# rcelha/rio-rs

Measured on NVIDIA H100. Metric: placements/sec, higher is better.
Workload: dtype u32

## Files before the change

rio_rs_b200/csrc/engine.cu:

```cuda
#include "../../include/rio_cuda.h"
#include "../../include/rio_cuda_dev.h"
#include "kernels.cuh"
#include "k_ranked.cuh"
#include "k_affinity_ranked.cuh"
#include "k_changes.cuh"
#include "k_ranked_changes.cuh"
#include "spec.cuh"
#include "trie_table.hpp"

#include <dlfcn.h>

#include <algorithm>
#include <atomic>
#include <chrono>
#include <cstdio>
#include <cstring>
#include <mutex>
#include <string>
#include <unordered_map>
#include <vector>

using namespace rio;

namespace {
// ... 190 lines not shown
    return h->h_scalars[which];
}
void check_device_error(rio_placement *h) {
    uint32_t e = 0;
    CUDA_TRY(cudaMemcpyAsync(&e, h->d_error(), 4, cudaMemcpyDeviceToHost, h->stream));
    CUDA_TRY(cudaStreamSynchronize(h->stream));
    if (e) { CUDA_TRY(cudaMemsetAsync(h->d_error(), 0, 4, h->stream)); throw RioError{RIO_ERR_UNKNOWN, "directory table overflow (internal sizing error)"}; }
}

bool address_malformed(const std::string &a) {
    size_t c = a.find(':');
    return c == std::string::npos || c == 0 || c + 1 >= a.size();
}

uint32_t intern_node(rio_placement *h, const std::string &addr) {
    auto it = h->node_index.find(addr);
    if (it != h->node_index.end()) return it->second;
    REQUIRE(h->nodes.size() < 0xFFFFFFF0u, "too many nodes");
    NodeInfo ni;
    ni.addr = addr;
    ni.seed = mix64(fnv1a64(addr.data(), addr.size()));
    ni.seed2 = mix64(ni.seed ^ kSaltNode2);
    ni.malformed = address_malformed(addr);
    uint32_t idx = (uint32_t)h->nodes.size();
    h->nodes.push_back(std::move(ni));
    h->node_index.emplace(addr, idx);
    h->tab_dirty = true;
    return idx;
}

void build_tab(rio_placement *h, TabBufs &tb, const std::vector<uint8_t> *closed) {
    const uint32_t n_total = (uint32_t)h->nodes.size();
    struct Ent { uint32_t invw, idx; };
    std::vector<Ent> live;
    auto is_closed = [&](uint32_t j) { return closed && j < closed->size() && (*closed)[j]; };
    for (uint32_t j = 0; j < n_total; j++) {
        const NodeInfo &ni = h->nodes[j];
        if (!ni.live()) continue;
        if (is_closed(j)) continue;
        live.push_back(Ent{inv_weight(ni.weight), j});
    }
    {
        std::vector<uint32_t> classes_seen;
        bool few = true;
        for (const Ent &e : live) {
            if (std::find(classes_seen.begin(), classes_seen.end(), e.invw) != classes_seen.end()) continue;
            if (classes_seen.size() == 64) { few = false; break; }
            classes_seen.push_back(e.invw);
        }
        if (few) {
            std::sort(classes_seen.begin(), classes_seen.end());
            std::vector<uint32_t> start(classes_seen.size() + 1, 0);
            auto cls = [&](uint32_t invw) { return (size_t)(std::lower_bound(classes_seen.begin(), classes_seen.end(), invw) - classes_seen.begin()); };
            for (const Ent &e : live) start[cls(e.invw) + 1]++;
            for (size_t c = 0; c < classes_seen.size(); c++) start[c + 1] += start[c];
            std::vector<Ent> grouped(live.size());
            for (const Ent &e : live) grouped[start[cls(e.invw)]++] = e;
            live.swap(grouped);
        } else {
            std::sort(live.begin(), live.end(), [](const Ent &a, const Ent &b) { return a.invw != b.invw ? a.invw < b.invw : a.idx < b.idx; });
        }
    }
    std::vector<NodeRec> recs(live.size() ? live.size() : 1);
    std::vector<ClassRec> classes;
    for (size_t q = 0; q < live.size(); q++) {
        const NodeInfo &ni = h->nodes[live[q].idx];
        recs[q] = NodeRec{(uint32_t)ni.seed, live[q].idx, (uint32_t)(ni.seed >> 32) | 1u, (uint32_t)ni.seed2};
        if (q == 0 || live[q].invw != live[q - 1].invw || (h->dev_table_flags & RIO_DEV_SPLIT_CLASSES)) classes.push_back(ClassRec{(uint32_t)q, live[q].invw});
    }
    const uint32_t n_classes = (uint32_t)classes.size();
    classes.push_back(ClassRec{(uint32_t)live.size(), 0});
    classes.push_back(ClassRec{(uint32_t)live.size(), 0});
    std::vector<uint4> by_idx(n_total ? n_total : 1);
    for (uint32_t j = 0; j < n_total; j++) {
        const NodeInfo &ni = h->nodes[j];
        const bool lv = ni.live() && !is_closed(j);
        by_idx[j] = make_uint4((uint32_t)ni.seed, lv ? inv_weight(ni.weight) : 0u, (uint32_t)(ni.seed >> 32) | 1u, (uint32_t)ni.seed2);
    }
    std::vector<TrieMember> members;
    members.reserve(live.size());
    for (const Ent &e : live) members.push_back(TrieMember{h->nodes[e.idx].seed, e.idx, h->nodes[e.idx].weight});
    const TrieBlob blob = build_trie_blob(members, h->trie_bits);
    const uint32_t bits = blob.bits, nb = 1u << bits, blob_bytes = blob.blob_bytes;
    std::vector<uint8_t> state(n_total ? n_total : 1, 0);
    std::vector<uint32_t> livef(n_total ? n_total : 1, 0);
    for (uint32_t j = 0; j < n_total; j++) {
        const NodeInfo &ni = h->nodes[j];
        state[j] = ((ni.active && !ni.malformed) ? kNodeLive : 0) | (ni.malformed ? kNodeMalformed : 0);
        livef[j] = ni.live() ? 1u : 0u;
    }

    auto al = [](size_t v) { return (v + 255) & ~(size_t)255; };
    const size_t o_recs = 0, o_classes = al(o_recs + recs.size() * sizeof(NodeRec)), o_byidx = al(o_classes + classes.size() * sizeof(ClassRec)),
                 o_trie = al(o_byidx + by_idx.size() * sizeof(uint4)), o_state = al(o_trie + blob_bytes), o_live = al(o_state + state.size()),
                 total = al(o_live + livef.size() * 4);
    cudaStream_t st = h->stream;
    if (tb.upload_pending) { CUDA_TRY(cudaStreamSynchronize(st)); tb.upload_pending = false; }
    if (h->aux_stream) CUDA_TRY(cudaStreamSynchronize(h->aux_stream));
    if (total > tb.stage_cap) {
        if (tb.stage) CUDA_TRY(cudaFreeHost(tb.stage));
        tb.stage = nullptr; tb.stage_cap = 0;
        CUDA_TRY(cudaMallocHost(reinterpret_cast<void **>(&tb.stage), total * 2));
        tb.stage_cap = total * 2;
    }
    memcpy(tb.stage + o_recs, recs.data(), recs.size() * sizeof(NodeRec));
    memcpy(tb.stage + o_classes, classes.data(), classes.size() * sizeof(ClassRec));
    memcpy(tb.stage + o_byidx, by_idx.data(), by_idx.size() * sizeof(uint4));
    memcpy(tb.stage + o_trie, blob.words.data(), blob_bytes);
    memcpy(tb.stage + o_state, state.data(), state.size());
    memcpy(tb.stage + o_live, livef.data(), livef.size() * 4);
    tb.dev.ensure(total, st);
    CUDA_TRY(cudaMemcpyAsync(tb.dev.p, tb.stage, total, cudaMemcpyHostToDevice, st));
    tb.upload_pending = true;
    unsigned char *d = tb.dev.as<unsigned char>();
    tb.trie = TrieDev{d + o_trie, blob_bytes, blob.off_crec, bits, blob.n_chain, {}};
    for (uint32_t i = 1; i < 8 && i < nb; i++) tb.trie.top[i] = blob.words[i];
    tb.tab.recs = reinterpret_cast<const NodeRec *>(d + o_recs);
    tb.tab.classes = reinterpret_cast<const ClassRec *>(d + o_classes);
    tb.tab.by_idx = reinterpret_cast<const uint4 *>(d + o_byidx);
    tb.tab.n_live = (uint32_t)live.size();
    tb.tab.n_classes = n_classes;
    tb.tab.n_total = n_total;
    tb.state = d + o_state;
    tb.live = reinterpret_cast<const uint32_t *>(d + o_live);
}

uint64_t live_signature(const rio_placement *h) {
    uint64_t sig = kFnvBasis;
    for (uint32_t j = 0; j < (uint32_t)h->nodes.size(); j++)
        if (h->nodes[j].live()) sig = mix64(sig ^ (((uint64_t)j << 32) | h->nodes[j].weight));
    return sig;
}

void ensure_tab(rio_placement *h) {
    if (!h->tab_dirty) return;
    build_tab(h, h->tabs, nullptr);
    const uint32_t n_total = (uint32_t)h->nodes.size();
    cudaStream_t st = h->stream;
    h->tab_dirty = false;
    h->tab_version++;
    h->live_sig = live_signature(h);
    if (!h->K) return;
    std::vector<float> fnode((size_t)(n_total ? n_total : 1) * h->K, 0.f);
    for (uint32_t j = 0; j < n_total; j++) {
        const NodeInfo &ni = h->nodes[j];
        if (ni.feat.size() == h->K) std::copy(ni.feat.begin(), ni.feat.end(), fnode.begin() + (size_t)j * h->K);
    }
    h->d_fnode.ensure(fnode.size() * 4, st);
    CUDA_TRY(cudaMemcpyAsync(h->d_fnode.p, fnode.data(), fnode.size() * 4, cudaMemcpyHostToDevice, st));
    h->aff_live = h->aff_pad = 0;
    if (h->K == 16) {
        std::vector<uint32_t> map;
        for (uint32_t j = 0; j < n_total; j++) if (h->nodes[j].live()) map.push_back(j);
        const uint32_t nl = (uint32_t)map.size();
        const uint32_t pad = nl <= 64 ? 64 : (nl + 255) / 256 * 256;
        std::vector<float> fc((size_t)pad * 16, 0.f);
        for (uint32_t q = 0; q < nl; q++) if (h->nodes[map[q]].feat.size() == 16) std::copy(h->nodes[map[q]].feat.begin(), h->nodes[map[q]].feat.end(), fc.begin() + (size_t)q * 16);
        map.resize(pad, kNone);
        std::vector<float> fg(fc.size());
        for (uint32_t g8 = 0; g8 < pad / 8; g8++)
            for (uint32_t k4 = 0; k4 < 4; k4++)
                for (uint32_t r8 = 0; r8 < 8; r8++)
                    std::copy_n(fc.begin() + ((size_t)g8 * 8 + r8) * 16 + k4 * 4, 4, fg.begin() + (((size_t)g8 * 4 + k4) * 8 + r8) * 4);
        h->d_fnode_c.ensure(fc.size() * 4, st);
        h->d_fnode_g.ensure(fg.size() * 4, st);
        CUDA_TRY(cudaMemcpyAsync(h->d_fnode_g.p, fg.data(), fg.size() * 4, cudaMemcpyHostToDevice, st));
        h->d_nidx_map.ensure(map.size() * 4, st);
        CUDA_TRY(cudaMemcpyAsync(h->d_fnode_c.p, fc.data(), fc.size() * 4, cudaMemcpyHostToDevice, st));
        CUDA_TRY(cudaMemcpyAsync(h->d_nidx_map.p, map.data(), map.size() * 4, cudaMemcpyHostToDevice, st));
        CUDA_TRY(cudaStreamSynchronize(st));
        h->aff_live = nl; h->aff_pad = pad;
    }
    CUDA_TRY(cudaStreamSynchronize(st));
}

uint64_t pow2_at_least(uint64_t v) { uint64_t p = 1; while (p < v) p <<= 1; return p; }

void dir_alloc(rio_placement *h, uint64_t cap, DirDev &out) {
    void *p = nullptr;
    CUDA_TRY(cudaMallocAsync(&p, cap * sizeof(DirSlot), h->stream));
    out.slots = reinterpret_cast<DirSlot *>(p);
    out.mask = cap - 1;
    uint32_t lg = 0; while ((1ull << lg) < cap) lg++;
    out.shift = 64 - lg;
    launch_dir_init(h->L(), out.slots, cap);
}

void reconcile_dir_keys(rio_placement *h) {
    h->dir_keys = read_scalar(h, S_NEWKEYS);
    h->dir_keys_pending = 0;
}

void dir_reserve(rio_placement *h, uint64_t n_more) {
    const uint64_t need = h->dir_keys + h->dir_keys_pending + n_more;
    if (need * 10 <= h->dir_cap * 7) return;
    if (h->dir_keys_pending) { reconcile_dir_keys(h); if ((h->dir_keys + n_more) * 10 <= h->dir_cap * 7) return; }
    zero_scalar(h, S_PLACED);
    launch_dir_count(h->L(), h->dir, h->d_scalars + S_PLACED, nullptr, 0);
// ... 1556 lines not shown
```

rio_rs_b200/csrc/k_trie.cu:

```cuda
#include "kernels.cuh"
#include "spec.cuh"
#include "bounded_tail.cuh"

#include <cstdlib>

namespace rio {

namespace {

#define RIO_COUNT_LAUNCH(L) do { if ((L).launch_counter) ++*(L).launch_counter; } while (0)

constexpr int kTrieThreads = 256;
constexpr uint32_t kMaxLevels = 16;

__constant__ uint32_t c_lvl_s0[kMaxLevels];
__constant__ uint32_t c_lvl_m2[kMaxLevels];
__constant__ uint32_t c_lvl_h2[kMaxLevels];

__device__ __forceinline__ uint32_t smem_u32(const void *p) { return (uint32_t)__cvta_generic_to_shared(p); }

__device__ __forceinline__ void stage_blob_tma(void *smem_dst, const void *gsrc, uint32_t bytes, unsigned long long *bar) {
    if (threadIdx.x == 0) {
        asm volatile("mbarrier.init.shared::cta.b64 [%0], 1;" ::"r"(smem_u32(bar)) : "memory");
        asm volatile("fence.mbarrier_init.release.cluster;" ::: "memory");
    }
    __syncthreads();
    if (threadIdx.x == 0) {
        asm volatile("mbarrier.arrive.expect_tx.shared::cta.b64 _, [%0], %1;" ::"r"(smem_u32(bar)), "r"(bytes) : "memory");
        for (uint32_t off = 0; off < bytes; off += 32768u) {
            const uint32_t len = min(32768u, bytes - off);
            asm volatile("cp.async.bulk.shared::cluster.global.mbarrier::complete_tx::bytes [%0], [%1], %2, [%3];"
                         ::"r"(smem_u32(reinterpret_cast<unsigned char *>(smem_dst) + off)),
                           "l"(reinterpret_cast<const unsigned char *>(gsrc) + off), "r"(len), "r"(smem_u32(bar))
                         : "memory");
        }
    }
    uint32_t done = 0;
    while (!done) {
        asm volatile("{\n\t.reg .pred p;\n\tmbarrier.try_wait.parity.shared::cta.b64 p, [%1], %2;\n\tselp.u32 %0, 1, 0, p;\n\t}"
                     : "=r"(done) : "r"(smem_u32(bar)), "r"(0u) : "memory");
    }
}

__device__ __forceinline__ uint32_t walk_step(uint32_t off, uint32_t sel) {
    uint32_t r;
    asm("mad.lo.u32 %0, %1, 2, %2;" : "=r"(r) : "r"(off), "r"(sel));
    return r;
}

template <int BITS>
__device__ __forceinline__ uint32_t trie_leaf_index(ObjHash o, const uint32_t *__restrict__ tab32, uint32_t bits_rt) {
    uint32_t i = 1;
    if (BITS > 0) {
#pragma unroll
        for (int l = 0; l < BITS; l++) {
            const uint32_t u = contest_u(o, c_lvl_s0[l], c_lvl_m2[l], c_lvl_h2[l]);
            i = 2 * i + (u > tab32[i] ? 1u : 0u);
        }
    } else {
        for (uint32_t l = 0; l < bits_rt; l++) {
            const uint32_t u = contest_u(o, c_lvl_s0[l], c_lvl_m2[l], c_lvl_h2[l]);
            i = 2 * i + (u > tab32[i] ? 1u : 0u);
        }
    }
    return i;
}

__device__ __forceinline__ uint32_t trie_resolve_leaf(ObjHash o, uint32_t leaf, const unsigned char *__restrict__ blob) {
    if ((int32_t)leaf > -2) return leaf;
    uint32_t w = leaf;
    for (;;) {
        const unsigned char *p = blob + (w & 0x7FFFFFFFu);
        const uint4 r = *reinterpret_cast<const uint4 *>(p);
        const uint2 nn = *reinterpret_cast<const uint2 *>(p + 16);
        if (contest_u(o, r.x, r.y, r.z) <= r.w) return nn.x;
        if ((int32_t)nn.y >= 0) return nn.y;
        w = nn.y;
    }
}

struct TrieSmem {
    const uint32_t *tab32;
    const unsigned char *blob;
    uint32_t *hist;
};

template <bool SMEM>
__device__ __forceinline__ TrieSmem trie_stage(const TrieDev &t, uint32_t hist_bins) {
    extern __shared__ __align__(128) unsigned char smem_trie[];
    constexpr bool in_smem = SMEM;
    TrieSmem s;
    uint32_t off = 0;
    if (in_smem) {
        s.tab32 = reinterpret_cast<const uint32_t *>(smem_trie);
        s.blob = smem_trie;
        off = t.blob_bytes;
    } else {
        const unsigned char *g = reinterpret_cast<const unsigned char *>(t.blob);
        s.tab32 = reinterpret_cast<const uint32_t *>(g);
        s.blob = g;
    }
    s.hist = reinterpret_cast<uint32_t *>(smem_trie + off);
    for (uint32_t j = threadIdx.x; j < hist_bins; j += blockDim.x) s.hist[j] = 0;
    unsigned long long *bar = reinterpret_cast<unsigned long long *>(smem_trie + off + ((hist_bins * 4u + 15u) & ~15u));
    if (in_smem) stage_blob_tma(smem_trie, t.blob, t.blob_bytes, bar);
    else __syncthreads();
    return s;
}

template <int BITS, int OPT, int MODE, bool SMEM, int MINB = (SMEM ? 5 : 3)>
__global__ void __launch_bounds__(kTrieThreads, MINB)
k_assign_trie(const uint64_t *__restrict__ keys, uint64_t n, TrieDev t, uint32_t *__restrict__ out_idx, uint32_t *__restrict__ counters,
              uint32_t hist_bins, unsigned long long *__restrict__ moved, const __grid_constant__ BoundedTail tail) {
    static_assert(OPT % 2 == 0, "two objects per 128-bit load");
    constexpr bool in_smem = SMEM;
    constexpr int SEG = OPT / 2;
    const uint64_t tile_objs = (uint64_t)kTrieThreads * OPT;
    const uint64_t n_tiles = (n + tile_objs - 1) / tile_objs;
    unsigned long long n_moved = 0;
    ulonglong2 kk[SEG];
    auto load_tile = [&](uint64_t tile) {
        const uint64_t f0 = tile * tile_objs + 2 * threadIdx.x;
        if ((tile + 1) * tile_objs <= n) {
            const ulonglong2 *src = reinterpret_cast<const ulonglong2 *>(keys + f0);
#pragma unroll
            for (int g = 0; g < SEG; g++) kk[g] = __ldg(src + g * kTrieThreads);
            return;
        }
#pragma unroll
        for (int g = 0; g < SEG; g++) {
            const uint64_t f = f0 + (uint64_t)g * (2 * kTrieThreads);
            kk[g] = make_ulonglong2(0, 0);
            if (f + 1 < n) kk[g] = __ldg(reinterpret_cast<const ulonglong2 *>(keys + f));
            else if (f < n) kk[g].x = __ldg(keys + f);
        }
    };
    const TrieSmem s = trie_stage<SMEM>(t, hist_bins);
    asm volatile("griddepcontrol.launch_dependents;" ::: "memory");
    asm volatile("griddepcontrol.wait;" ::: "memory");
    if (blockIdx.x < n_tiles) load_tile(blockIdx.x);
    for (uint64_t tile = blockIdx.x; tile < n_tiles; tile += gridDim.x) {
        const uint64_t base = tile * tile_objs;
        const bool full_tile = base + tile_objs <= n;
        ObjHash o[OPT];
#pragma unroll
        for (int g = 0; g < SEG; g++) {
            o[2 * g] = obj_hash(kk[g].x);
            o[2 * g + 1] = obj_hash(kk[g].y);
        }
        if (tile + gridDim.x < n_tiles) load_tile(tile + gridDim.x);
        uint32_t leaf[OPT];
        if (in_smem) {
            const unsigned char *tb = reinterpret_cast<const unsigned char *>(s.tab32);
            uint32_t off[OPT];
#pragma unroll
            for (int k = 0; k < OPT; k++) off[k] = 4;
            if (BITS > 0) {
                constexpr int TOP = BITS >= 3 ? 3 : 0;
                if (TOP) {
#pragma unroll
                    for (int k = 0; k < OPT; k++) {
                        const bool c0 = contest_u(o[k], c_lvl_s0[0], c_lvl_m2[0], c_lvl_h2[0]) > t.top[1];
                        const bool c1 = contest_u(o[k], c_lvl_s0[1], c_lvl_m2[1], c_lvl_h2[1]) > (c0 ? t.top[3] : t.top[2]);
                        const uint32_t t2 = c0 ? (c1 ? t.top[7] : t.top[6]) : (c1 ? t.top[5] : t.top[4]);
                        const bool c2 = contest_u(o[k], c_lvl_s0[2], c_lvl_m2[2], c_lvl_h2[2]) > t2;
                        off[k] = 32u + (c0 ? 16u : 0u) + (c1 ? 8u : 0u) + (c2 ? 4u : 0u);
                    }
                }
#pragma unroll
                for (int l = TOP; l < BITS; l++) {
#pragma unroll
                    for (int k = 0; k < OPT; k++) {
                        const uint32_t u = contest_u(o[k], c_lvl_s0[l], c_lvl_m2[l], c_lvl_h2[l]);
                        const uint32_t thr = *reinterpret_cast<const uint32_t *>(tb + off[k]);
                        off[k] = walk_step(off[k], u > thr ? 4u : 0u);
                    }
                }
            } else {
                for (uint32_t l = 0; l < t.bits; l++) {
#pragma unroll
                    for (int k = 0; k < OPT; k++) {
                        const uint32_t u = contest_u(o[k], c_lvl_s0[l], c_lvl_m2[l], c_lvl_h2[l]);
                        const uint32_t thr = *reinterpret_cast<const uint32_t *>(tb + off[k]);
                        off[k] = walk_step(off[k], u > thr ? 4u : 0u);
                    }
                }
            }
#pragma unroll
            for (int k = 0; k < OPT; k++) leaf[k] = *reinterpret_cast<const uint32_t *>(tb + off[k]);
        } else {
#pragma unroll
            for (int k = 0; k < OPT; k++) leaf[k] = __ldg(s.tab32 + trie_leaf_index<0>(o[k], s.tab32, t.bits));
        }
        uint32_t nid[OPT];
#pragma unroll
        for (int k = 0; k < OPT; k++) nid[k] = trie_resolve_leaf(o[k], leaf[k], s.blob);
        if (MODE == 0 && full_tile) {
            uint2 *dst = reinterpret_cast<uint2 *>(out_idx + base + 2 * threadIdx.x);
#pragma unroll
            for (int g = 0; g < SEG; g++) dst[g * kTrieThreads] = make_uint2(nid[2 * g], nid[2 * g + 1]);
            if (counters && nid[0] != kNone) {
                if (hist_bins) {
#pragma unroll
                    for (int k = 0; k < OPT; k++) atomicAdd(&s.hist[nid[k]], 1u);
                } else {
#pragma unroll
                    for (int k = 0; k < OPT; k++) atomicAdd(&counters[nid[k]], 1u);
                }
            }
            continue;
        }
#pragma unroll
        for (int g = 0; g < SEG; g++) {
            const uint64_t first = base + (uint64_t)g * (2 * kTrieThreads) + 2 * threadIdx.x;
            if (first >= n) continue;
            const bool two = first + 1 < n;
            if (MODE == 1) {
                uint2 old = make_uint2(kNone, kNone);
                if (two) old = *reinterpret_cast<const uint2 *>(out_idx + first);
                else old.x = out_idx[first];
                const bool c0 = old.x != nid[2 * g], c1 = two && old.y != nid[2 * g + 1];
                if (c0 | c1) {
                    if (two) *reinterpret_cast<uint2 *>(out_idx + first) = make_uint2(nid[2 * g], nid[2 * g + 1]);
                    else out_idx[first] = nid[2 * g];
                }
                n_moved += (unsigned)c0 + (unsigned)c1;
            } else {
                if (two) *reinterpret_cast<uint2 *>(out_idx + first) = make_uint2(nid[2 * g], nid[2 * g + 1]);
                else out_idx[first] = nid[2 * g];
            }
            if (counters) {
                if (hist_bins) {
                    if (nid[2 * g] != kNone) atomicAdd(&s.hist[nid[2 * g]], 1u);
                    if (two && nid[2 * g + 1] != kNone) atomicAdd(&s.hist[nid[2 * g + 1]], 1u);
                } else {
                    if (nid[2 * g] != kNone) atomicAdd(&counters[nid[2 * g]], 1u);
                    if (two && nid[2 * g + 1] != kNone) atomicAdd(&counters[nid[2 * g + 1]], 1u);
                }
            }
        }
    }
    if (MODE == 1) {
#pragma unroll
        for (int sh = 16; sh > 0; sh >>= 1) n_moved += __shfl_xor_sync(0xFFFFFFFFu, n_moved, sh);
        if ((threadIdx.x & 31) == 0 && n_moved) atomicAdd(moved, n_moved);
    }
    if (hist_bins && counters) {
        __syncthreads();
        for (uint32_t j = threadIdx.x; j < hist_bins; j += blockDim.x) { const uint32_t v = s.hist[j]; if (v) atomicAdd(&counters[j], v); }
    }
    if (MODE == 0 && tail.enabled) {
        __shared__ uint32_t s_last;
        __threadfence();
        __syncthreads();
        if (threadIdx.x == 0) s_last = atomicAdd(tail.ticket, 1u) == gridDim.x - 1;
        __syncthreads();
        if (s_last) {
            if (threadIdx.x == 0) *tail.ticket = 0;
            __threadfence();
            exchange_and_check_block(tail, counters);
        }
    }
}

template <bool SMEM>
__global__ void __launch_bounds__(kTrieThreads, 4)
k_assign_trie_sel(const uint64_t *__restrict__ keys, const uint32_t *__restrict__ sel, uint64_t n_sel, TrieDev t, uint32_t *__restrict__ out_idx,
                  uint32_t *__restrict__ counters, uint32_t hist_bins) {
    const TrieSmem s = trie_stage<SMEM>(t, hist_bins);
    for (uint64_t q = (uint64_t)blockIdx.x * blockDim.x + threadIdx.x; q < n_sel; q += (uint64_t)gridDim.x * blockDim.x) {
        const uint32_t oi = __ldg(sel + q);
        const ObjHash o = obj_hash(__ldg(keys + oi));
        const uint32_t i = trie_leaf_index<0>(o, s.tab32, t.bits);
        const uint32_t nid = trie_resolve_leaf(o, s.tab32[i], s.blob);
        out_idx[oi] = nid;
        if (counters && nid != kNone) { if (hist_bins) atomicAdd(&s.hist[nid], 1u); else atomicAdd(&counters[nid], 1u); }
    }
    if (hist_bins && counters) {
        __syncthreads();
        for (uint32_t j = threadIdx.x; j < hist_bins; j += blockDim.x) { const uint32_t v = s.hist[j]; if (v) atomicAdd(&counters[j], v); }
    }
}

template <bool SMEM>
__global__ void __launch_bounds__(kTrieThreads, 4)
k_dir_reassign_trie(DirDev dir, TrieDev t, unsigned long long *__restrict__ moved) {
    const TrieSmem s = trie_stage<SMEM>(t, 0);
    const uint4 *slots = reinterpret_cast<const uint4 *>(dir.slots);
    const uint64_t cap = dir.mask + 1;
    unsigned long long n_moved = 0;
    for (uint64_t i = (uint64_t)blockIdx.x * blockDim.x + threadIdx.x; i < cap; i += (uint64_t)gridDim.x * blockDim.x) {
        const uint4 v = slots[i];
        const unsigned long long key = ((unsigned long long)v.y << 32) | v.x;
        if (key == kEmptyKey || v.z == kNone) continue;
        const ObjHash o = obj_hash(key);
        const uint32_t li = trie_leaf_index<0>(o, s.tab32, t.bits);
        const uint32_t nid = trie_resolve_leaf(o, s.tab32[li], s.blob);
        if (nid != v.z) { reinterpret_cast<uint32_t *>(&dir.slots[i].val)[0] = nid; n_moved++; }
    }
#pragma unroll
    for (int sh = 16; sh > 0; sh >>= 1) n_moved += __shfl_xor_sync(0xFFFFFFFFu, n_moved, sh);
    if ((threadIdx.x & 31) == 0 && n_moved) atomicAdd(moved, n_moved);
}

constexpr uint32_t kTrieSmemBudget = 200u * 1024u;

struct TrieLaunchShape { uint32_t hist_bins; uint32_t in_smem; size_t smem; int ctas_per_sm; };
TrieLaunchShape trie_shape(const TrieDev &t, bool want_hist, uint32_t n_total, int want_ctas) {
    TrieLaunchShape sh{};
    sh.hist_bins = (want_hist && n_total <= 8192) ? n_total : 0;
    const size_t tail = ((size_t)sh.hist_bins * 4 + 15) / 16 * 16 + 16;
    sh.in_smem = (t.blob_bytes + tail <= kTrieSmemBudget) ? 1u : 0u;
    sh.smem = (sh.in_smem ? t.blob_bytes : 0) + tail;
    int c = want_ctas;
    while (c > 1 && (size_t)c * (sh.smem + 1024) > 227u * 1024u) c--;
    sh.ctas_per_sm = c;
    return sh;
}

bool g_lvl_uploaded[64] = {};

}

void trie_upload_level_constants(int device) {
    if (device >= 0 && device < 64 && g_lvl_uploaded[device]) return;
    uint32_t s0[kMaxLevels], m2[kMaxLevels], h2[kMaxLevels];
    for (uint32_t l = 0; l < kMaxLevels; l++) {
        const ContestRec r = contest_rec(level_seed(l));
        s0[l] = r.s0; m2[l] = r.m2; h2[l] = r.h2;
    }
    cudaMemcpyToSymbol(c_lvl_s0, s0, sizeof s0);
    cudaMemcpyToSymbol(c_lvl_m2, m2, sizeof m2);
    cudaMemcpyToSymbol(c_lvl_h2, h2, sizeof h2);
    if (device >= 0 && device < 64) g_lvl_uploaded[device] = true;
}

uint64_t trie_wave_objects(int sm_count) { return (uint64_t)sm_count * 5 * kTrieThreads * 4; }

#define RIO_TRIE_LAUNCH(KERNEL, GRID, SMEM, ...)                                                                       \
    do {                                                                                                               \
        static bool attr_set[64] = {};    \
        int dev__ = 0;                                                                                                 \
        cudaGetDevice(&dev__);                                                                                         \
        if (dev__ < 0 || dev__ >= 64 || !attr_set[dev__]) {                                                            \
            cudaFuncSetAttribute(KERNEL, cudaFuncAttributeMaxDynamicSharedMemorySize, (int)kTrieSmemBudget + 1024);    \
            if (dev__ >= 0 && dev__ < 64) attr_set[dev__] = true;                                                      \
        }                                                                                                              \
        KERNEL<<<(GRID), kTrieThreads, (SMEM), L.stream>>>(__VA_ARGS__);                                               \
    } while (0)

#define RIO_TRIE_LAUNCH_PDL(KERNEL, GRID, SMEM, ...)                                                                   \
    do {                                                                                                               \
        static bool attr_set[64] = {};                                                                                 \
        static const bool pdl = [] { const char *e = getenv("RIO_TRIE_PDL"); return !(e && e[0] == '0'); }();          \
        int dev__ = 0;                                                                                                 \
        cudaGetDevice(&dev__);                                                                                         \
        if (dev__ < 0 || dev__ >= 64 || !attr_set[dev__]) {                                                            \
            cudaFuncSetAttribute(KERNEL, cudaFuncAttributeMaxDynamicSharedMemorySize, (int)kTrieSmemBudget + 1024);    \
            if (dev__ >= 0 && dev__ < 64) attr_set[dev__] = true;                                                      \
        }                                                                                                              \
        cudaLaunchConfig_t cfg__ = {};                                                                                 \
        cfg__.gridDim = dim3((unsigned)(GRID)); cfg__.blockDim = dim3(kTrieThreads);                                   \
        cfg__.dynamicSmemBytes = (SMEM); cfg__.stream = L.stream;                                                      \
        cudaLaunchAttribute at__[1];                                                                                   \
        at__[0].id = cudaLaunchAttributeProgrammaticStreamSerialization;                                               \
        at__[0].val.programmaticStreamSerializationAllowed = 1;                                                        \
        cfg__.attrs = at__; cfg__.numAttrs = pdl ? 1 : 0;                                                              \
        cudaLaunchKernelEx(&cfg__, KERNEL, __VA_ARGS__);                                                               \
    } while (0)

void launch_assign_trie(const Launch &L, const uint64_t *d_keys, uint64_t n, const TrieDev &t, uint32_t *d_out_idx, uint32_t *d_counters,
                        const uint32_t *d_sel, uint64_t n_sel, uint32_t n_total, const BoundedTail *tail) {
    BoundedTail no_tail{};
    const BoundedTail &tl = tail ? *tail : no_tail;
    const uint64_t n_work = d_sel ? n_sel : n;
    if (!n_work) return;
    if (d_sel) {
        const TrieLaunchShape sh = trie_shape(t, d_counters != nullptr, n_total, 4);
        const uint64_t blocks = (n_work + kTrieThreads - 1) / kTrieThreads, cap = (uint64_t)L.sm_count * sh.ctas_per_sm;
        const int grid = (int)(blocks < cap ? blocks : cap);
        if (sh.in_smem) RIO_TRIE_LAUNCH(k_assign_trie_sel<true>, grid, sh.smem, d_keys, d_sel, n_work, t, d_out_idx, d_counters, sh.hist_bins);
        else RIO_TRIE_LAUNCH(k_assign_trie_sel<false>, grid, sh.smem, d_keys, d_sel, n_work, t, d_out_idx, d_counters, sh.hist_bins);
    } else {
        constexpr int OPT = 4;
#ifdef RIO_ASSIGN_TUNING
        if (const char *tn = getenv("RIO_TRIE_TUNE")) {
            const int code = atoi(tn);
            auto go = [&](auto kern, int opt, int minb) {
                const TrieLaunchShape sh2 = trie_shape(t, d_counters != nullptr, n_total, minb);
                const uint64_t tiles2 = (n_work + (uint64_t)kTrieThreads * opt - 1) / ((uint64_t)kTrieThreads * opt), cap2 = (uint64_t)L.sm_count * sh2.ctas_per_sm;
                cudaFuncSetAttribute(kern, cudaFuncAttributeMaxDynamicSharedMemorySize, (int)kTrieSmemBudget + 1024);
                kern<<<(int)(tiles2 < cap2 ? tiles2 : cap2), kTrieThreads, sh2.smem, L.stream>>>(d_keys, n_work, t, d_out_idx, d_counters, sh2.hist_bins, nullptr, tl);
            };
            bool done = true;
            switch (code) {
                case 25: go(k_assign_trie<12, 2, 0, true, 5>, 2, 5); break;
                case 28: go(k_assign_trie<12, 2, 0, true, 8>, 2, 8); break;
                case 44: go(k_assign_trie<12, 4, 0, true, 4>, 4, 4); break;
                case 45: go(k_assign_trie<12, 4, 0, true, 5>, 4, 5); break;
                case 63: go(k_assign_trie<12, 6, 0, true, 3>, 6, 3); break;
                case 64: go(k_assign_trie<12, 6, 0, true, 4>, 6, 4); break;
                case 83: go(k_assign_trie<12, 8, 0, true, 3>, 8, 3); break;
                default: done = false;
            }
            if (done && t.bits == 12) { RIO_COUNT_LAUNCH(L); return; }
        }
#endif
        const TrieLaunchShape sh = trie_shape(t, d_counters != nullptr, n_total, 5);
        uint64_t cap = (uint64_t)L.sm_count * sh.ctas_per_sm;
        if (L.spare_ctas > 0 && cap > (uint64_t)L.spare_ctas + 1) cap -= (uint64_t)L.spare_ctas;
        const uint64_t tiles = (n_work + (uint64_t)kTrieThreads * OPT - 1) / ((uint64_t)kTrieThreads * OPT);
        const int grid = (int)(tiles < cap ? tiles : cap);
        unsigned long long *no_moved = nullptr;
        if (!sh.in_smem) RIO_TRIE_LAUNCH_PDL((k_assign_trie<0, OPT, 0, false>), grid, sh.smem, d_keys, n_work, t, d_out_idx, d_counters, sh.hist_bins, no_moved, tl);
        else if (t.bits == 12) RIO_TRIE_LAUNCH_PDL((k_assign_trie<12, OPT, 0, true>), grid, sh.smem, d_keys, n_work, t, d_out_idx, d_counters, sh.hist_bins, no_moved, tl);
        else RIO_TRIE_LAUNCH_PDL((k_assign_trie<0, OPT, 0, true>), grid, sh.smem, d_keys, n_work, t, d_out_idx, d_counters, sh.hist_bins, no_moved, tl);
    }
    RIO_COUNT_LAUNCH(L);
}

void launch_reassign_trie(const Launch &L, const uint64_t *d_keys, uint64_t n, const TrieDev &t, uint32_t *d_idx, uint32_t *d_counters,
                          uint32_t n_total, unsigned long long *d_moved) {
    if (!n) return;
    constexpr int OPT = 4;
 const TrieLaunchShape sh = trie_shape(t, d_counters != nullptr, n_total, 5);
    const uint64_t tiles = (n + (uint64_t)kTrieThreads * OPT - 1) / ((uint64_t)kTrieThreads * OPT), cap = (uint64_t)L.sm_count * sh.ctas_per_sm;
    const int grid = (int)(tiles < cap ? tiles : cap);
    if (!sh.in_smem) RIO_TRIE_LAUNCH((k_assign_trie<0, OPT, 1, false>), grid, sh.smem, d_keys, n, t, d_idx, d_counters, sh.hist_bins, d_moved, BoundedTail{});
    else if (t.bits == 12) RIO_TRIE_LAUNCH((k_assign_trie<12, OPT, 1, true>), grid, sh.smem, d_keys, n, t, d_idx, d_counters, sh.hist_bins, d_moved, BoundedTail{});
    else RIO_TRIE_LAUNCH((k_assign_trie<0, OPT, 1, true>), grid, sh.smem, d_keys, n, t, d_idx, d_counters, sh.hist_bins, d_moved, BoundedTail{});
    RIO_COUNT_LAUNCH(L);
}

void launch_dir_reassign_trie(const Launch &L, const DirDev &dir, const TrieDev &t, unsigned long long *d_moved) {
    const TrieLaunchShape sh = trie_shape(t, false, 0, 4);
    const uint64_t blocks = (dir.mask + 1 + kTrieThreads - 1) / kTrieThreads, cap = (uint64_t)L.sm_count * sh.ctas_per_sm;
    const int grid = (int)(blocks < cap ? blocks : cap);
    if (sh.in_smem) RIO_TRIE_LAUNCH(k_dir_reassign_trie<true>, grid, sh.smem, dir, t, d_moved);
    else RIO_TRIE_LAUNCH(k_dir_reassign_trie<false>, grid, sh.smem, dir, t, d_moved);
    RIO_COUNT_LAUNCH(L);
}

}
```

rio_rs_b200/csrc/kernels.cuh:

```cuda
#pragma once
#include <cuda_runtime.h>
#include <cstdint>

namespace rio {

struct __align__(16) NodeRec {
    uint32_t s0;
    uint32_t nidx;
    uint32_t s1;
    uint32_t s2;
};
struct ClassRec {
    uint32_t start;
    uint32_t invw;
};
struct NodeTabDev {
    const NodeRec *recs;
    const ClassRec *classes;
    uint32_t n_live;
    uint32_t n_classes;
    uint32_t n_total;
    const uint4 *by_idx;
};

struct TrieDev {
    const void *blob;
    uint32_t blob_bytes;
    uint32_t off_crec;
    uint32_t bits;
    uint32_t n_chain;
    uint32_t top[8];
};

struct __align__(16) DirSlot {
    unsigned long long key;
    unsigned long long val;
};
constexpr unsigned long long kEmptyKey = 0xFFFFFFFFFFFFFFFFull;
constexpr unsigned long long kEmptyVal = 0x00000000FFFFFFFFull;
struct DirDev {
    DirSlot *slots;
    uint64_t mask;
    uint32_t shift;
};

struct Launch { cudaStream_t stream; int sm_count; uint64_t *launch_counter; int spare_ctas = 0;  };

struct XchgPeers { uint32_t *win[16]; };
struct BoundedTail {
    uint32_t enabled;
    uint32_t M;
    uint32_t *ticket;
    uint32_t *next_zero;
    XchgPeers peers;
    uint32_t rank, world, max_nodes, xchg_epoch;
    uint32_t *glob;
    const uint32_t *cap;
    const uint8_t *state;
    uint32_t *closed_epoch;
    uint32_t call_epoch;
    uint32_t *thr;
    uint8_t *over;
    volatile uint32_t *host_flags;
    uint32_t flag_seq;
};

void launch_assign_hrw(const Launch &L, const uint64_t *d_keys, uint64_t n, const NodeTabDev &tab, uint32_t *d_out_idx,
                       uint32_t *d_counters , const uint32_t *d_sel , uint64_t n_sel);
uint64_t assign_wave_objects(int sm_count);
void trie_upload_level_constants(int device);
uint64_t trie_wave_objects(int sm_count);
void launch_assign_affinity(const Launch &L, const float *d_fobj, uint64_t n, const float *d_fnode ,
                            const uint32_t *d_live , uint32_t n_total, uint32_t K, uint32_t *d_out_idx,
                            float *d_out_cost , uint32_t *d_counters);
uint32_t affinity_umma_max_nodes();
void affinity_umma_set_timing_buffer(unsigned long long *d);
cudaError_t launch_assign_affinity_umma(const Launch &L, const float *d_fobj, uint64_t n, const float *d_fnode_c, const float *d_fnode_g, const uint32_t *d_nidx_map, uint32_t n_live,
                                 uint32_t m_pad, uint32_t n_total, uint32_t *d_out_idx, float *d_out_cost, uint32_t *d_counters);
uint64_t launch_mix_rate(const Launch &L, uint32_t iters, uint32_t *d_sink);
void launch_synth_keys(const Launch &L, uint64_t *d_keys, uint64_t first, uint64_t n, uint64_t seed);
void launch_hash_ids(const Launch &L, const char *d_packed, const uint64_t *d_offsets, uint64_t n, uint64_t *d_keys);
void launch_fill_u32(const Launch &L, uint32_t *d, uint64_t n, uint32_t v);
void launch_histogram(const Launch &L, const uint32_t *d_idx, uint64_t n, uint32_t *d_counters, uint32_t n_total);

void launch_select_spill(const Launch &L, const uint64_t *d_keys, const uint32_t *d_idx, uint64_t n, const uint32_t *d_thr ,
                         const uint8_t *d_over, uint32_t round, uint32_t *d_sel, unsigned long long *d_nsel, uint32_t *d_counters);

void launch_rebalance_join(const Launch &L, const uint64_t *d_keys, uint32_t *d_idx, uint64_t n, const NodeTabDev &tab, uint32_t new_idx,
                           uint32_t *d_counters, unsigned long long *d_moved);
void launch_select_on_node(const Launch &L, const uint32_t *d_idx, uint64_t n, uint32_t node, uint32_t *d_sel, unsigned long long *d_nsel);

void launch_dir_init(const Launch &L, DirSlot *slots, uint64_t cap);
void launch_dir_lookup(const Launch &L, const DirDev &dir, const uint64_t *d_keys, uint64_t n, uint32_t *d_out);
void launch_dir_upsert(const Launch &L, const DirDev &dir, const uint64_t *d_keys, const uint32_t *d_idx , uint32_t const_idx,
                       uint64_t n, uint32_t seq_base, unsigned long long *d_new_keys, uint32_t *d_error);
void launch_dir_clear_seq(const Launch &L, const DirDev &dir);
void launch_dir_clean_node(const Launch &L, const DirDev &dir, uint32_t node, unsigned long long *d_removed);
void launch_dir_clean_flagged(const Launch &L, const DirDev &dir, const uint8_t *d_flag, uint32_t n_total, unsigned long long *d_removed);
void launch_dir_rehash(const Launch &L, const DirDev &from, const DirDev &to, unsigned long long *d_new_keys, uint32_t *d_error);
void launch_dir_count(const Launch &L, const DirDev &dir, unsigned long long *d_placed, uint32_t *d_counters , uint32_t n_total);
void launch_dir_rebalance_join(const Launch &L, const DirDev &dir, const NodeTabDev &tab, uint32_t new_idx, unsigned long long *d_moved);
void launch_dir_rebalance_leave(const Launch &L, const DirDev &dir, const NodeTabDev &tab, uint32_t gone_idx, unsigned long long *d_moved);

void launch_assign_trie(const Launch &L, const uint64_t *d_keys, uint64_t n, const TrieDev &t, uint32_t *d_out_idx, uint32_t *d_counters ,
                        const uint32_t *d_sel , uint64_t n_sel, uint32_t n_total, const BoundedTail *tail = nullptr);
void launch_reassign_trie(const Launch &L, const uint64_t *d_keys, uint64_t n, const TrieDev &t, uint32_t *d_idx, uint32_t *d_counters ,
                          uint32_t n_total, unsigned long long *d_moved);
void launch_dir_reassign_trie(const Launch &L, const DirDev &dir, const TrieDev &t, unsigned long long *d_moved);

void launch_classify(const Launch &L, const uint32_t *d_cur, uint64_t n, const uint8_t *d_node_state, uint32_t n_total, uint32_t *d_sel,
                     unsigned long long *d_nsel, uint8_t *d_dead_flag);
void launch_check_address(const Launch &L, const uint32_t *d_idx, uint64_t n, const uint8_t *d_verdict_tab, uint32_t n_total, uint8_t *d_out, uint8_t *d_dead_flag,
                          unsigned long long *d_ndead);
void launch_scatter_const(const Launch &L, uint32_t *d_out, const uint32_t *d_sel, uint64_t n_sel, uint32_t v);
// ... 13 lines not shown
```

rio_rs_b200/csrc/trie_table.hpp:

```cpp
#pragma once
#include <algorithm>
#include <cstdint>
#include <memory>
#include <vector>

#include "spec.cuh"

namespace rio {

struct TrieMember {
    uint64_t seed;
    uint32_t idx;
    uint32_t weight;
};

struct TrieBlob {
    std::vector<uint32_t> words;
    uint32_t blob_bytes = 0;
    uint32_t off_crec = 0;
    uint32_t n_chain = 0;
    uint32_t bits = 0;
    std::vector<uint64_t> wsum;
};

// ... 7 lines not shown
    while (q * s > num) q--;
    while ((q + 1) * s <= num) q++;
    return q ? (uint32_t)(2 * q - 1) : 0u;
}

inline TrieBlob build_trie_blob(const std::vector<TrieMember> &members, uint32_t bits) {
    const uint32_t nb = 1u << bits;
    struct Mem { uint64_t pos; uint64_t seed; uint32_t idx, w; };
    std::vector<uint32_t> bstart((size_t)nb + 1, 0);
    std::vector<Mem> all;
    all.reserve(members.size());
    for (const TrieMember &m : members) {
        if (!m.weight) continue;
        const uint64_t pos = mix64(m.seed ^ kSaltPos);
        all.push_back(Mem{pos, m.seed, m.idx, m.weight});
        bstart[(bits ? (uint32_t)(pos >> (64 - bits)) : 0u) + 1]++;
    }
    for (uint32_t k = 0; k < nb; k++) bstart[k + 1] += bstart[k];
    std::unique_ptr<Mem[]> mem(new Mem[all.size() ? all.size() : 1]);
    {
        std::vector<uint32_t> fill(bstart.begin(), bstart.end() - 1);
        for (const Mem &m : all) mem[fill[bits ? (uint32_t)(m.pos >> (64 - bits)) : 0u]++] = m;
    }
    std::vector<uint64_t> wsum((size_t)2 * nb, 0);
    uint32_t n_rec = 0;
    for (uint32_t k = 0; k < nb; k++) {
        const uint32_t lo = bstart[k], hi = bstart[k + 1];
        if (hi - lo > 1) {
            std::sort(mem.get() + lo, mem.get() + hi, [](const Mem &a, const Mem &b) { return a.pos != b.pos ? a.pos < b.pos : a.idx < b.idx; });
            n_rec += hi - lo - 1;
        }
        uint64_t sum = 0;
        for (uint32_t q = lo; q < hi; q++) sum += mem[q].w;
        wsum[nb + k] = sum;
    }
    for (uint32_t i = nb - 1; i >= 1; i--) wsum[i] = wsum[2 * i] + wsum[2 * i + 1];
    TrieBlob b;
    b.bits = bits;
    b.off_crec = (uint32_t)(((size_t)2 * nb * 4 + 15) / 16 * 16);
    b.n_chain = n_rec;
    b.blob_bytes = std::max<uint32_t>(16u, b.off_crec + n_rec * 32u);
    b.words.assign(b.blob_bytes / 4, 0u);
    uint32_t *w32 = b.words.data();
    for (uint32_t i = 1; i < nb; i++) w32[i] = contest_t3_fast(wsum[2 * i], wsum[2 * i + 1]);
    uint32_t rec_off = b.off_crec;
    for (uint32_t k = 0; k < nb; k++) {
        const uint32_t lo = bstart[k], hi = bstart[k + 1];
        if (lo == hi) { w32[nb + k] = kNone; continue; }
        if (hi - lo == 1) { w32[nb + k] = mem[lo].idx; continue; }
        w32[nb + k] = 0x80000000u | rec_off;
        uint64_t rest = wsum[nb + k];
        for (uint32_t q = lo; q + 1 < hi; q++, rec_off += 32u) {
            rest -= mem[q].w;
            const ContestRec r = contest_rec(mem[q].seed);
            uint32_t *d = w32 + rec_off / 4;
            d[0] = r.s0; d[1] = r.m2; d[2] = r.h2; d[3] = contest_t3_fast(mem[q].w, rest);
            d[4] = mem[q].idx;
            d[5] = q + 2 == hi ? mem[hi - 1].idx : 0x80000000u | (rec_off + 32u);
        }
    }
    b.wsum = std::move(wsum);
    return b;
}

inline std::vector<ContestRec> trie_level_constants(uint32_t levels) {
    std::vector<ContestRec> v(levels);
    for (uint32_t l = 0; l < levels; l++) v[l] = contest_rec(level_seed(l));
    return v;
}

inline uint32_t trie_walk_host(const uint32_t *blob, uint32_t bits, const ContestRec *level, ObjHash o) {
    uint32_t i = 1;
    for (uint32_t l = 0; l < bits; l++) i = 2 * i + (contest_u(o, level[l].s0, level[l].m2, level[l].h2) > blob[i] ? 1u : 0u);
    uint32_t w = blob[i];
    if ((int32_t)w > -2) return w;
    for (;;) {
        const uint32_t *p = blob + (w & 0x7FFFFFFFu) / 4;
        if (contest_u(o, p[0], p[1], p[2]) <= p[3]) return p[4];
        if ((int32_t)p[5] >= 0) return p[5];
        w = p[5];
    }
}

}
```

Baseline: 162.6 billion.

## Pack trie levels in pairs into one word with exact global fallback on ties

Builds a packed trie table where each word holds truncated thresholds for a node and both of its children. The kernel then walks two levels per shared-memory load instead of one. Walks that come close to a truncated threshold are detected per warp and redone with the exact thresholds from global memory. Only the leaf portion of the original blob is staged next to the packed table, which cuts the number of dependent smem loads in the walk. In exchange it adds a divergent fallback path, extra host-side packing and a larger upload.

```diff
diff --git a/rio_rs_b200/csrc/engine.cu b/rio_rs_b200/csrc/engine.cu
--- a/rio_rs_b200/csrc/engine.cu
+++ b/rio_rs_b200/csrc/engine.cu
@@ -296,6 +296,7 @@
     for (const Ent &e : live) members.push_back(TrieMember{h->nodes[e.idx].seed, e.idx, h->nodes[e.idx].weight});
     const TrieBlob blob = build_trie_blob(members, h->trie_bits);
     const uint32_t bits = blob.bits, nb = 1u << bits, blob_bytes = blob.blob_bytes;
+    const std::vector<uint32_t> pack = trie_pack(blob);
     std::vector<uint8_t> state(n_total ? n_total : 1, 0);
     std::vector<uint32_t> livef(n_total ? n_total : 1, 0);
     for (uint32_t j = 0; j < n_total; j++) {
@@ -306,7 +307,8 @@
 
     auto al = [](size_t v) { return (v + 255) & ~(size_t)255; };
     const size_t o_recs = 0, o_classes = al(o_recs + recs.size() * sizeof(NodeRec)), o_byidx = al(o_classes + classes.size() * sizeof(ClassRec)),
-                 o_trie = al(o_byidx + by_idx.size() * sizeof(uint4)), o_state = al(o_trie + blob_bytes), o_live = al(o_state + state.size()),
+                 o_trie = al(o_byidx + by_idx.size() * sizeof(uint4)), o_pack = al(o_trie + blob_bytes), o_state = al(o_pack + pack.size() * 4),
+                 o_live = al(o_state + state.size()),
                  total = al(o_live + livef.size() * 4);
     cudaStream_t st = h->stream;
     if (tb.upload_pending) { CUDA_TRY(cudaStreamSynchronize(st)); tb.upload_pending = false; }
@@ -321,13 +323,14 @@
     memcpy(tb.stage + o_classes, classes.data(), classes.size() * sizeof(ClassRec));
     memcpy(tb.stage + o_byidx, by_idx.data(), by_idx.size() * sizeof(uint4));
     memcpy(tb.stage + o_trie, blob.words.data(), blob_bytes);
+    memcpy(tb.stage + o_pack, pack.data(), pack.size() * 4);
     memcpy(tb.stage + o_state, state.data(), state.size());
     memcpy(tb.stage + o_live, livef.data(), livef.size() * 4);
     tb.dev.ensure(total, st);
     CUDA_TRY(cudaMemcpyAsync(tb.dev.p, tb.stage, total, cudaMemcpyHostToDevice, st));
     tb.upload_pending = true;
     unsigned char *d = tb.dev.as<unsigned char>();
-    tb.trie = TrieDev{d + o_trie, blob_bytes, blob.off_crec, bits, blob.n_chain, {}};
+    tb.trie = TrieDev{d + o_trie, blob_bytes, blob.off_crec, bits, blob.n_chain, {}, d + o_pack, (uint32_t)pack.size() * 4};
     for (uint32_t i = 1; i < 8 && i < nb; i++) tb.trie.top[i] = blob.words[i];
     tb.tab.recs = reinterpret_cast<const NodeRec *>(d + o_recs);
     tb.tab.classes = reinterpret_cast<const ClassRec *>(d + o_classes);
diff --git a/rio_rs_b200/csrc/k_trie.cu b/rio_rs_b200/csrc/k_trie.cu
--- a/rio_rs_b200/csrc/k_trie.cu
+++ b/rio_rs_b200/csrc/k_trie.cu
@@ -1,6 +1,7 @@
 #include "kernels.cuh"
 #include "spec.cuh"
 #include "bounded_tail.cuh"
+#include "trie_table.hpp"
 
 #include <cstdlib>
 
@@ -19,21 +20,27 @@
 
 __device__ __forceinline__ uint32_t smem_u32(const void *p) { return (uint32_t)__cvta_generic_to_shared(p); }
 
-__device__ __forceinline__ void stage_blob_tma(void *smem_dst, const void *gsrc, uint32_t bytes, unsigned long long *bar) {
+__device__ __forceinline__ void bulk_copy_chunks(void *smem_dst, const void *gsrc, uint32_t bytes, unsigned long long *bar) {
+    for (uint32_t off = 0; off < bytes; off += 32768u) {
+        const uint32_t len = min(32768u, bytes - off);
+        asm volatile("cp.async.bulk.shared::cluster.global.mbarrier::complete_tx::bytes [%0], [%1], %2, [%3];"
+                     ::"r"(smem_u32(reinterpret_cast<unsigned char *>(smem_dst) + off)),
+                       "l"(reinterpret_cast<const unsigned char *>(gsrc) + off), "r"(len), "r"(smem_u32(bar))
+                     : "memory");
+    }
+}
+
+__device__ __forceinline__ void stage_blob_tma(void *smem_dst, const void *gsrc, uint32_t bytes, unsigned long long *bar,
+                                               const void *gsrc1 = nullptr, uint32_t bytes1 = 0) {
     if (threadIdx.x == 0) {
         asm volatile("mbarrier.init.shared::cta.b64 [%0], 1;" ::"r"(smem_u32(bar)) : "memory");
         asm volatile("fence.mbarrier_init.release.cluster;" ::: "memory");
     }
     __syncthreads();
     if (threadIdx.x == 0) {
-        asm volatile("mbarrier.arrive.expect_tx.shared::cta.b64 _, [%0], %1;" ::"r"(smem_u32(bar)), "r"(bytes) : "memory");
-        for (uint32_t off = 0; off < bytes; off += 32768u) {
-            const uint32_t len = min(32768u, bytes - off);
-            asm volatile("cp.async.bulk.shared::cluster.global.mbarrier::complete_tx::bytes [%0], [%1], %2, [%3];"
-                         ::"r"(smem_u32(reinterpret_cast<unsigned char *>(smem_dst) + off)),
-                           "l"(reinterpret_cast<const unsigned char *>(gsrc) + off), "r"(len), "r"(smem_u32(bar))
-                         : "memory");
-        }
+        asm volatile("mbarrier.arrive.expect_tx.shared::cta.b64 _, [%0], %1;" ::"r"(smem_u32(bar)), "r"(bytes + bytes1) : "memory");
+        bulk_copy_chunks(smem_dst, gsrc, bytes, bar);
+        if (bytes1) bulk_copy_chunks(reinterpret_cast<unsigned char *>(smem_dst) + bytes, gsrc1, bytes1, bar);
     }
     uint32_t done = 0;
     while (!done) {
@@ -48,6 +55,25 @@
     return r;
 }
 
+__device__ __forceinline__ uint32_t pair_step(uint32_t off, uint32_t w, uint32_t u0, uint32_t u1, uint32_t &dist) {
+    const bool c0 = u0 > w;
+    const uint32_t f = w << (c0 ? 21 : 10);
+    const bool c1 = u1 > f;
+    dist = __vimin3_u32(dist, (u0 ^ w) >> 1, u1 ^ f);
+    return 4u * off + (c0 ? 8u : 0u) + (c1 ? 4u : 0u);
+}
+
+__device__ __forceinline__ uint32_t trie_rewalk_pairs(ObjHash o, uint32_t i, uint32_t p0, uint32_t bits, const uint32_t *__restrict__ g32) {
+#pragma unroll 1
+    for (uint32_t l = p0; l < bits; l += 2) {
+        const uint32_t t0 = __ldg(g32 + i), tl = __ldg(g32 + 2 * i), tr = __ldg(g32 + 2 * i + 1);
+        const bool c0 = contest_u(o, c_lvl_s0[l], c_lvl_m2[l], c_lvl_h2[l]) > t0;
+        const bool c1 = contest_u(o, c_lvl_s0[l + 1], c_lvl_m2[l + 1], c_lvl_h2[l + 1]) > (c0 ? tr : tl);
+        i = 4 * i + (c0 ? 2u : 0u) + (c1 ? 1u : 0u);
+    }
+    return i;
+}
+
 template <int BITS>
 __device__ __forceinline__ uint32_t trie_leaf_index(ObjHash o, const uint32_t *__restrict__ tab32, uint32_t bits_rt) {
     uint32_t i = 1;
@@ -66,11 +92,11 @@
     return i;
 }
 
-__device__ __forceinline__ uint32_t trie_resolve_leaf(ObjHash o, uint32_t leaf, const unsigned char *__restrict__ blob) {
+__device__ __forceinline__ uint32_t trie_resolve_leaf(ObjHash o, uint32_t leaf, const unsigned char *__restrict__ blob, uint32_t rebase = 0) {
     if ((int32_t)leaf > -2) return leaf;
     uint32_t w = leaf;
     for (;;) {
-        const unsigned char *p = blob + (w & 0x7FFFFFFFu);
+        const unsigned char *p = blob + ((w & 0x7FFFFFFFu) + rebase);
         const uint4 r = *reinterpret_cast<const uint4 *>(p);
         const uint2 nn = *reinterpret_cast<const uint2 *>(p + 16);
         if (contest_u(o, r.x, r.y, r.z) <= r.w) return nn.x;
@@ -82,19 +108,23 @@
 struct TrieSmem {
     const uint32_t *tab32;
     const unsigned char *blob;
+    uint32_t rebase;
     uint32_t *hist;
 };
 
-template <bool SMEM>
+template <bool SMEM, bool PACKED = false>
 __device__ __forceinline__ TrieSmem trie_stage(const TrieDev &t, uint32_t hist_bins) {
     extern __shared__ __align__(128) unsigned char smem_trie[];
     constexpr bool in_smem = SMEM;
     TrieSmem s;
+    s.rebase = 0;
     uint32_t off = 0;
+    const uint32_t lo = PACKED ? trie_leaf_lo(t.bits) : 0u;
     if (in_smem) {
         s.tab32 = reinterpret_cast<const uint32_t *>(smem_trie);
         s.blob = smem_trie;
-        off = t.blob_bytes;
+        off = PACKED ? t.pack_bytes + (t.blob_bytes - lo) : t.blob_bytes;
+        if (PACKED) s.rebase = t.pack_bytes - lo;
     } else {
         const unsigned char *g = reinterpret_cast<const unsigned char *>(t.blob);
         s.tab32 = reinterpret_cast<const uint32_t *>(g);
@@ -103,7 +133,8 @@
     s.hist = reinterpret_cast<uint32_t *>(smem_trie + off);
     for (uint32_t j = threadIdx.x; j < hist_bins; j += blockDim.x) s.hist[j] = 0;
     unsigned long long *bar = reinterpret_cast<unsigned long long *>(smem_trie + off + ((hist_bins * 4u + 15u) & ~15u));
-    if (in_smem) stage_blob_tma(smem_trie, t.blob, t.blob_bytes, bar);
+    if (in_smem && PACKED) stage_blob_tma(smem_trie, t.pack, t.pack_bytes, bar, reinterpret_cast<const unsigned char *>(t.blob) + lo, t.blob_bytes - lo);
+    else if (in_smem) stage_blob_tma(smem_trie, t.blob, t.blob_bytes, bar);
     else __syncthreads();
     return s;
 }
@@ -135,7 +166,7 @@
             else if (f < n) kk[g].x = __ldg(keys + f);
         }
     };
-    const TrieSmem s = trie_stage<SMEM>(t, hist_bins);
+    const TrieSmem s = trie_stage<SMEM, true>(t, hist_bins);
     asm volatile("griddepcontrol.launch_dependents;" ::: "memory");
     asm volatile("griddepcontrol.wait;" ::: "memory");
     if (blockIdx.x < n_tiles) load_tile(blockIdx.x);
@@ -152,9 +183,9 @@
         uint32_t leaf[OPT];
         if (in_smem) {
             const unsigned char *tb = reinterpret_cast<const unsigned char *>(s.tab32);
-            uint32_t off[OPT];
-#pragma unroll
-            for (int k = 0; k < OPT; k++) off[k] = 4;
+            uint32_t off[OPT], dist[OPT];
+#pragma unroll
+            for (int k = 0; k < OPT; k++) { off[k] = 4; dist[k] = 0xFFFFFFFFu; }
             if (BITS > 0) {
                 constexpr int TOP = BITS >= 3 ? 3 : 0;
                 if (TOP) {
@@ -167,8 +198,9 @@
                         off[k] = 32u + (c0 ? 16u : 0u) + (c1 ? 8u : 0u) + (c2 ? 4u : 0u);
                     }
                 }
-#pragma unroll
-                for (int l = TOP; l < BITS; l++) {
+                constexpr int P0 = (int)trie_pair_from(BITS);
+#pragma unroll
+                for (int l = TOP; l < P0; l++) {
 #pragma unroll
                     for (int k = 0; k < OPT; k++) {
                         const uint32_t u = contest_u(o[k], c_lvl_s0[l], c_lvl_m2[l], c_lvl_h2[l]);
@@ -176,8 +208,18 @@
                         off[k] = walk_step(off[k], u > thr ? 4u : 0u);
                     }
                 }
+#pragma unroll
+                for (int l = P0; l < BITS; l += 2) {
+#pragma unroll
+                    for (int k = 0; k < OPT; k++) {
+                        const uint32_t u0 = contest_u(o[k], c_lvl_s0[l], c_lvl_m2[l], c_lvl_h2[l]);
+                        const uint32_t u1 = contest_u(o[k], c_lvl_s0[l + 1], c_lvl_m2[l + 1], c_lvl_h2[l + 1]);
+                        off[k] = pair_step(off[k], *reinterpret_cast<const uint32_t *>(tb + off[k]), u0, u1, dist[k]);
+                    }
+                }
             } else {
-                for (uint32_t l = 0; l < t.bits; l++) {
+                const uint32_t p0 = trie_pair_from(t.bits);
+                for (uint32_t l = 0; l < p0; l++) {
 #pragma unroll
                     for (int k = 0; k < OPT; k++) {
                         const uint32_t u = contest_u(o[k], c_lvl_s0[l], c_lvl_m2[l], c_lvl_h2[l]);
@@ -185,16 +227,33 @@
                         off[k] = walk_step(off[k], u > thr ? 4u : 0u);
                     }
                 }
+                for (uint32_t l = p0; l < t.bits; l += 2) {
+#pragma unroll
+                    for (int k = 0; k < OPT; k++) {
+                        const uint32_t u0 = contest_u(o[k], c_lvl_s0[l], c_lvl_m2[l], c_lvl_h2[l]);
+                        const uint32_t u1 = contest_u(o[k], c_lvl_s0[l + 1], c_lvl_m2[l + 1], c_lvl_h2[l + 1]);
+                        off[k] = pair_step(off[k], *reinterpret_cast<const uint32_t *>(tb + off[k]), u0, u1, dist[k]);
+                    }
+                }
             }
-#pragma unroll
-            for (int k = 0; k < OPT; k++) leaf[k] = *reinterpret_cast<const uint32_t *>(tb + off[k]);
+            bool tie = false;
+#pragma unroll
+            for (int k = 0; k < OPT; k++) tie |= dist[k] < kTrieTie;
+            if (__any_sync(0xFFFFFFFFu, tie)) {
+                const uint32_t bits = BITS > 0 ? (uint32_t)BITS : t.bits, p0 = trie_pair_from(bits);
+#pragma unroll
+                for (int k = 0; k < OPT; k++)
+                    if (dist[k] < kTrieTie) off[k] = 4u * trie_rewalk_pairs(o[k], (off[k] >> 2) >> (bits - p0), p0, bits, reinterpret_cast<const uint32_t *>(t.blob));
+            }
+#pragma unroll
+            for (int k = 0; k < OPT; k++) leaf[k] = *reinterpret_cast<const uint32_t *>(tb + (off[k] + s.rebase));
         } else {
 #pragma unroll
             for (int k = 0; k < OPT; k++) leaf[k] = __ldg(s.tab32 + trie_leaf_index<0>(o[k], s.tab32, t.bits));
         }
         uint32_t nid[OPT];
 #pragma unroll
-        for (int k = 0; k < OPT; k++) nid[k] = trie_resolve_leaf(o[k], leaf[k], s.blob);
+        for (int k = 0; k < OPT; k++) nid[k] = trie_resolve_leaf(o[k], leaf[k], s.blob, s.rebase);
         if (MODE == 0 && full_tile) {
             uint2 *dst = reinterpret_cast<uint2 *>(out_idx + base + 2 * threadIdx.x);
 #pragma unroll
@@ -306,12 +365,13 @@
 constexpr uint32_t kTrieSmemBudget = 200u * 1024u;
 
 struct TrieLaunchShape { uint32_t hist_bins; uint32_t in_smem; size_t smem; int ctas_per_sm; };
-TrieLaunchShape trie_shape(const TrieDev &t, bool want_hist, uint32_t n_total, int want_ctas) {
+TrieLaunchShape trie_shape(const TrieDev &t, bool want_hist, uint32_t n_total, int want_ctas, bool packed = false) {
     TrieLaunchShape sh{};
     sh.hist_bins = (want_hist && n_total <= 8192) ? n_total : 0;
     const size_t tail = ((size_t)sh.hist_bins * 4 + 15) / 16 * 16 + 16;
     sh.in_smem = (t.blob_bytes + tail <= kTrieSmemBudget) ? 1u : 0u;
-    sh.smem = (sh.in_smem ? t.blob_bytes : 0) + tail;
+    const size_t staged = packed ? (size_t)t.pack_bytes + t.blob_bytes - trie_leaf_lo(t.bits) : t.blob_bytes;
+    sh.smem = (sh.in_smem ? staged : 0) + tail;
     int c = want_ctas;
     while (c > 1 && (size_t)c * (sh.smem + 1024) > 227u * 1024u) c--;
     sh.ctas_per_sm = c;
@@ -387,7 +447,7 @@
         if (const char *tn = getenv("RIO_TRIE_TUNE")) {
             const int code = atoi(tn);
             auto go = [&](auto kern, int opt, int minb) {
-                const TrieLaunchShape sh2 = trie_shape(t, d_counters != nullptr, n_total, minb);
+                const TrieLaunchShape sh2 = trie_shape(t, d_counters != nullptr, n_total, minb, true);
                 const uint64_t tiles2 = (n_work + (uint64_t)kTrieThreads * opt - 1) / ((uint64_t)kTrieThreads * opt), cap2 = (uint64_t)L.sm_count * sh2.ctas_per_sm;
                 cudaFuncSetAttribute(kern, cudaFuncAttributeMaxDynamicSharedMemorySize, (int)kTrieSmemBudget + 1024);
                 kern<<<(int)(tiles2 < cap2 ? tiles2 : cap2), kTrieThreads, sh2.smem, L.stream>>>(d_keys, n_work, t, d_out_idx, d_counters, sh2.hist_bins, nullptr, tl);
@@ -406,7 +466,7 @@
             if (done && t.bits == 12) { RIO_COUNT_LAUNCH(L); return; }
         }
 #endif
-        const TrieLaunchShape sh = trie_shape(t, d_counters != nullptr, n_total, 5);
+        const TrieLaunchShape sh = trie_shape(t, d_counters != nullptr, n_total, 5, true);
         uint64_t cap = (uint64_t)L.sm_count * sh.ctas_per_sm;
         if (L.spare_ctas > 0 && cap > (uint64_t)L.spare_ctas + 1) cap -= (uint64_t)L.spare_ctas;
         const uint64_t tiles = (n_work + (uint64_t)kTrieThreads * OPT - 1) / ((uint64_t)kTrieThreads * OPT);
@@ -423,7 +483,7 @@
                           uint32_t n_total, unsigned long long *d_moved) {
     if (!n) return;
     constexpr int OPT = 4;
- const TrieLaunchShape sh = trie_shape(t, d_counters != nullptr, n_total, 5);
+    const TrieLaunchShape sh = trie_shape(t, d_counters != nullptr, n_total, 5, true);
     const uint64_t tiles = (n + (uint64_t)kTrieThreads * OPT - 1) / ((uint64_t)kTrieThreads * OPT), cap = (uint64_t)L.sm_count * sh.ctas_per_sm;
     const int grid = (int)(tiles < cap ? tiles : cap);
     if (!sh.in_smem) RIO_TRIE_LAUNCH((k_assign_trie<0, OPT, 1, false>), grid, sh.smem, d_keys, n, t, d_idx, d_counters, sh.hist_bins, d_moved, BoundedTail{});
diff --git a/rio_rs_b200/csrc/kernels.cuh b/rio_rs_b200/csrc/kernels.cuh
--- a/rio_rs_b200/csrc/kernels.cuh
+++ b/rio_rs_b200/csrc/kernels.cuh
@@ -30,6 +30,8 @@
     uint32_t bits;
     uint32_t n_chain;
     uint32_t top[8];
+    const void *pack;
+    uint32_t pack_bytes;
 };
 
 struct __align__(16) DirSlot {
diff --git a/rio_rs_b200/csrc/trie_table.hpp b/rio_rs_b200/csrc/trie_table.hpp
--- a/rio_rs_b200/csrc/trie_table.hpp
+++ b/rio_rs_b200/csrc/trie_table.hpp
@@ -113,4 +113,56 @@
     }
 }
 
+RIO_HD constexpr uint32_t trie_pair_from(uint32_t bits) { return bits < 6u ? bits : 6u + ((bits - 6u) & 1u); }
+RIO_HD uint32_t trie_pack_bytes(uint32_t bits) {
+    const uint32_t words = 1u << (trie_pair_from(bits) < bits ? bits - 1u : bits);
+    return (4u * words + 15u) & ~15u;
 }
+RIO_HD uint32_t trie_leaf_lo(uint32_t bits) { return (4u << bits) & ~15u; }
+RIO_HD uint32_t trie_pack_word(uint32_t t, uint32_t tl, uint32_t tr) { return (t >> 22) << 22 | (tl >> 21) << 11 | (tr >> 21); }
+constexpr uint32_t kTrieTie = 1u << 21;
+
+inline std::vector<uint32_t> trie_pack(const TrieBlob &b) {
+    const uint32_t bits = b.bits, p0 = trie_pair_from(bits);
+    const uint32_t *t3 = b.words.data();
+    std::vector<uint32_t> p(trie_pack_bytes(bits) / 4, 0u);
+    for (uint32_t i = 1; i < (1u << p0); i++) p[i] = t3[i];
+    for (uint32_t l = p0; l < bits; l += 2)
+        for (uint32_t i = 1u << l; i < (2u << l); i++) p[i] = trie_pack_word(t3[i], t3[2 * i], t3[2 * i + 1]);
+    return p;
+}
+
+inline uint32_t trie_walk_packed_host(const uint32_t *pack, const uint32_t *blob, uint32_t bits, const ContestRec *level, ObjHash o) {
+    const uint32_t p0 = trie_pair_from(bits);
+    uint32_t i = 1, m = 0xFFFFFFFFu;
+    for (uint32_t l = 0; l < p0; l++) i = 2 * i + (contest_u(o, level[l].s0, level[l].m2, level[l].h2) > pack[i] ? 1u : 0u);
+    for (uint32_t l = p0; l < bits; l += 2) {
+        const uint32_t u0 = contest_u(o, level[l].s0, level[l].m2, level[l].h2);
+        const uint32_t u1 = contest_u(o, level[l + 1].s0, level[l + 1].m2, level[l + 1].h2);
+        const uint32_t w = pack[i];
+        const bool c0 = u0 > w;
+        const uint32_t f = w << (c0 ? 21 : 10);
+        const bool c1 = u1 > f;
+        m = std::min(m, std::min((u0 ^ w) >> 1, u1 ^ f));
+        i = 4 * i + (c0 ? 2u : 0u) + (c1 ? 1u : 0u);
+    }
+    if (m < kTrieTie) {
+        i >>= bits - p0;
+        for (uint32_t l = p0; l < bits; l += 2) {
+            const uint32_t t0 = blob[i], tl = blob[2 * i], tr = blob[2 * i + 1];
+            const bool c0 = contest_u(o, level[l].s0, level[l].m2, level[l].h2) > t0;
+            const bool c1 = contest_u(o, level[l + 1].s0, level[l + 1].m2, level[l + 1].h2) > (c0 ? tr : tl);
+            i = 4 * i + (c0 ? 2u : 0u) + (c1 ? 1u : 0u);
+        }
+    }
+    uint32_t w = blob[i];
+    if ((int32_t)w > -2) return w;
+    for (;;) {
+        const uint32_t *p = blob + (w & 0x7FFFFFFFu) / 4;
+        if (contest_u(o, p[0], p[1], p[2]) <= p[3]) return p[4];
+        if ((int32_t)p[5] >= 0) return p[5];
+        w = p[5];
+    }
+}
+
+}
```

After: 130.7 billion (median of 6 runs). 19.6% lower.
